# snuspl/parallax

Measured on NVIDIA H100. Metric: lm1b_words_per_sec, higher is better.
Workload: dtype bf16

## Files before the change

### parallax_b200/ops/csrc/kernels/gemm_tc.cu

```cuda
#include "wgmma.cuh"

namespace tc {

template <int BN, int STAGES>
__device__ __forceinline__ void mainloop(const CUtensorMap* tmap_a, const CUtensorMap* tmap_b,
                                         uint8_t* smem, uint64_t* full_bar, uint64_t* empty_bar,
                                         int k0, int num_kb, int m0, int n0, float* acc) {
  constexpr int A_BYTES = BM * BK * 2, B_BYTES = BN * BK * 2, STAGE_BYTES = A_BYTES + B_BYTES;
  const int wg = threadIdx.x >> 7;
  if (wg == 0) {
    if (threadIdx.x == 0) {
      for (int kb = 0; kb < num_kb; ++kb) {
        const int s = kb % STAGES;
        const uint32_t ph = (kb / STAGES) & 1;
        mbar_wait(&empty_bar[s], ph ^ 1);
        uint8_t* sa = smem + s * STAGE_BYTES;
        mbar_expect_tx(&full_bar[s], STAGE_BYTES);
        tma_load_2d(sa, tmap_a, &full_bar[s], k0 + kb * BK, m0);
        tma_load_2d(sa + A_BYTES, tmap_b, &full_bar[s], k0 + kb * BK, n0);
      }
    }
    return;
  }
  const int cw = wg - 1;
  const bool leader = (threadIdx.x & 127) == 0;
  for (int kb = 0; kb < num_kb; ++kb) {
    const int s = kb % STAGES;
    mbar_wait(&full_bar[s], (kb / STAGES) & 1);
    const uint32_t sa = smem_u32(smem + s * STAGE_BYTES);
    const uint64_t adesc = make_smem_desc(sa + cw * 64 * BK * 2);
    const uint64_t bdesc = make_smem_desc(sa + A_BYTES);
    wgmma_fence();
#pragma unroll
    for (int k = 0; k < BK / WG_K; ++k)
      wgmma_bf16<BN>(acc, adesc + (uint64_t)(k * 2), bdesc + (uint64_t)(k * 2),
                     (kb | k) != 0 ? 1u : 0u);
    wgmma_commit();
    wgmma_wait<1>();
    if (kb > 0 && leader) mbar_arrive(&empty_bar[(kb - 1) % STAGES]);
  }
  wgmma_wait<0>();
}

struct GemmArgs {
  __nv_bfloat16* C;
  const __nv_bfloat16* addend;
  float* ws;
  unsigned int* tickets;
  int M, N, K;
  int k_per_split;
};

__device__ __forceinline__ float2 bf16x2_to_float2(uint32_t w) {
  return make_float2(__uint_as_float(w << 16), __uint_as_float(w & 0xffff0000u));
}
__device__ __forceinline__ uint32_t float2_to_bf16x2(float a, float b) {
  __nv_bfloat162 h = __floats2bfloat162_rn(a, b);
  return *reinterpret_cast<uint32_t*>(&h);
}

__device__ __forceinline__ void cluster_sync_all() {
  asm volatile("barrier.cluster.arrive.release.aligned;\n"
               "barrier.cluster.wait.acquire.aligned;" ::: "memory");
}

template <int BN, int STAGES, bool CLUSTER>
__global__ void __launch_bounds__(THREADS, 1)
px_gemm_tc_kernel(const __grid_constant__ CUtensorMap tmap_a,
                  const __grid_constant__ CUtensorMap tmap_b, GemmArgs g) {
  extern __shared__ __align__(1024) uint8_t smem_raw[];
  uint8_t* smem = reinterpret_cast<uint8_t*>(((uintptr_t)smem_raw + 1023) & ~(uintptr_t)1023);
  constexpr int STAGE_BYTES = BM * BK * 2 + BN * BK * 2;
  uint64_t* full_bar = reinterpret_cast<uint64_t*>(smem + STAGES * STAGE_BYTES);
  uint64_t* empty_bar = full_bar + STAGES;
  __shared__ unsigned int s_last;

  const int n_tile = blockIdx.x, m_tile = blockIdx.y, split = blockIdx.z;

  if (threadIdx.x == 0) {
    asm volatile("prefetch.tensormap [%0];" ::"l"(&tmap_a) : "memory");
    asm volatile("prefetch.tensormap [%0];" ::"l"(&tmap_b) : "memory");
    for (int s = 0; s < STAGES; ++s) { mbar_init(&full_bar[s], 1); mbar_init(&empty_bar[s], 2); }
    asm volatile("fence.mbarrier_init.release.cluster;" ::: "memory");
  }
  __syncthreads();

  float acc[BN / 2];
  mainloop<BN, STAGES>(&tmap_a, &tmap_b, smem, full_bar, empty_bar, split * g.k_per_split,
                       g.k_per_split / BK, m_tile * BM, n_tile * BN, acc);

  if (threadIdx.x >= 128) {
    const int t = threadIdx.x - 128, lane = t & 31;
    const int lrow = (t >> 5) * 16 + (lane >> 2);
    const int lcol = (lane & 3) * 2;
    const bool splitk = gridDim.z > 1;
    if (CLUSTER) {
      consumer_sync();
      float* park = reinterpret_cast<float*>(smem);
#pragma unroll
      for (int j = 0; j < BN / 8; ++j)
#pragma unroll
        for (int h = 0; h < 2; ++h)
          *reinterpret_cast<float2*>(park + (size_t)(lrow + 8 * h) * (BN + 4) + j * 8 + lcol) =
              make_float2(acc[j * 4 + 2 * h], acc[j * 4 + 2 * h + 1]);
    } else {
#pragma unroll
      for (int h = 0; h < 2; ++h) {
        const int row = m_tile * BM + lrow + 8 * h;
        if (row >= g.M) continue;
        const size_t base = (size_t)row * g.N + (size_t)n_tile * BN + lcol;
#pragma unroll
        for (int j = 0; j < BN / 8; ++j) {
          const size_t off = base + j * 8;
          float2 v = make_float2(acc[j * 4 + 2 * h], acc[j * 4 + 2 * h + 1]);
          if (splitk) {
            atomicAdd(reinterpret_cast<float2*>(g.ws + off), v);
          } else {
            if (g.addend) {
              const float2 a = bf16x2_to_float2(*reinterpret_cast<const uint32_t*>(g.addend + off));
              v.x += a.x; v.y += a.y;
            }
            *reinterpret_cast<uint32_t*>(g.C + off) = float2_to_bf16x2(v.x, v.y);
          }
        }
      }
    }
  }
  __syncthreads();
  if (CLUSTER) {
    uint32_t crank, csize;
    asm volatile("mov.u32 %0, %%cluster_ctarank;" : "=r"(crank));
    asm volatile("mov.u32 %0, %%cluster_nctarank;" : "=r"(csize));
    cluster_sync_all();
    const int rows_per = BM / (int)csize;
    const int nvec = rows_per * BN / 4;
    const uint32_t my_base = smem_u32(smem);
    for (int v = threadIdx.x; v < nvec; v += blockDim.x) {
      const int rr = (int)crank * rows_per + (v * 4) / BN, cc = (v * 4) % BN;
      const uint32_t off_b = (uint32_t)(((size_t)rr * (BN + 4) + cc) * 4);
      float4 acc4 = make_float4(0.f, 0.f, 0.f, 0.f);
      for (uint32_t p = 0; p < csize; ++p) {
        uint32_t raddr;
        asm volatile("mapa.shared::cluster.u32 %0, %1, %2;" : "=r"(raddr) : "r"(my_base + off_b), "r"(p));
        float4 x;
        asm volatile("ld.shared::cluster.v4.f32 {%0,%1,%2,%3}, [%4];"
                     : "=f"(x.x), "=f"(x.y), "=f"(x.z), "=f"(x.w) : "r"(raddr) : "memory");
        acc4.x += x.x; acc4.y += x.y; acc4.z += x.z; acc4.w += x.w;
      }
      const int row = m_tile * BM + rr;
      if (row < g.M) {
        const size_t off = (size_t)row * g.N + (size_t)n_tile * BN + cc;
        if (g.addend) {
          const uint2 a2 = *reinterpret_cast<const uint2*>(g.addend + off);
          const float2 lo = bf16x2_to_float2(a2.x), hi = bf16x2_to_float2(a2.y);
          acc4.x += lo.x; acc4.y += lo.y; acc4.z += hi.x; acc4.w += hi.y;
        }
        *reinterpret_cast<uint2*>(g.C + off) =
            make_uint2(float2_to_bf16x2(acc4.x, acc4.y), float2_to_bf16x2(acc4.z, acc4.w));
      }
    }
    cluster_sync_all();
    return;
  }
  if (gridDim.z > 1) {
    __threadfence();
    __syncthreads();
    const unsigned int tile_id = m_tile * gridDim.x + n_tile;
    if (threadIdx.x == 0) s_last = (atomicAdd(&g.tickets[tile_id], 1u) == gridDim.z - 1) ? 1u : 0u;
    __syncthreads();
    if (s_last) {
      __threadfence();
      for (int idx = threadIdx.x; idx < BM * BN / 8; idx += blockDim.x) {
        const int rr = idx / (BN / 8), cc = (idx % (BN / 8)) * 8;
        const int row = m_tile * BM + rr;
        if (row >= g.M) continue;
        const size_t off = (size_t)row * g.N + (size_t)n_tile * BN + cc;
        float f[8];
        const uint4 lo = __ldcg(reinterpret_cast<const uint4*>(g.ws + off));
        const uint4 hi = __ldcg(reinterpret_cast<const uint4*>(g.ws + off + 4));
        f[0] = __uint_as_float(lo.x); f[1] = __uint_as_float(lo.y); f[2] = __uint_as_float(lo.z);
        f[3] = __uint_as_float(lo.w); f[4] = __uint_as_float(hi.x); f[5] = __uint_as_float(hi.y);
        f[6] = __uint_as_float(hi.z); f[7] = __uint_as_float(hi.w);
        if (g.addend) {
          float a[8];
          Vec16<__nv_bfloat16>::unpack(ld_v4(g.addend + off), a);
#pragma unroll
          for (int j = 0; j < 8; ++j) f[j] += a[j];
        }
        st_v4(g.C + off, Vec16<__nv_bfloat16>::pack(f));
        __stcg(reinterpret_cast<uint4*>(g.ws + off), make_uint4(0, 0, 0, 0));
        __stcg(reinterpret_cast<uint4*>(g.ws + off + 4), make_uint4(0, 0, 0, 0));
      }
      if (threadIdx.x == 0) g.tickets[tile_id] = 0;
    }
  }
}


template <int BN, int STAGES>
constexpr int smem_bytes() { return STAGES * (BM * BK * 2 + BN * BK * 2) + 1024 + 256; }

}

extern "C" {

int px_gemm_tc(const void* A, const void* B, void* C, const void* addend, float* ws,
               unsigned int* tickets, int M, int N, int K, int splits, int bn, int cluster,
               cudaStream_t stream) {
  using namespace tc;
  if (M % BM || K % BK || (bn != 64 && bn != 128) || N % bn) return -1;
  if (splits < 1 || K % (splits * BK)) return -2;
  if (cluster && (splits < 2 || splits > 16 || (BM % splits) != 0)) return -4;
  if (splits > 1 && !cluster && (!ws || !tickets)) return -3;
  CUtensorMap ta, tb;
  int rc = make_tmap(&ta, A, M, K, BM);
  if (rc) return rc;
  rc = make_tmap(&tb, B, N, K, bn);
  if (rc) return rc;
  GemmArgs g;
  g.C = (__nv_bfloat16*)C; g.addend = (const __nv_bfloat16*)addend; g.ws = ws;
  g.tickets = tickets; g.M = M; g.N = N; g.K = K; g.k_per_split = K / splits;
  dim3 grid(N / bn, M / BM, splits);
  constexpr int STAGES = 4;
  if (cluster) {
    cudaLaunchConfig_t cfg = {};
    cfg.gridDim = grid; cfg.blockDim = dim3(THREADS); cfg.stream = stream;
    cudaLaunchAttribute at[1];
    at[0].id = cudaLaunchAttributeClusterDimension;
    at[0].val.clusterDim.x = 1; at[0].val.clusterDim.y = 1; at[0].val.clusterDim.z = splits;
    cfg.attrs = at; cfg.numAttrs = 1;
    cudaError_t e;
    if (bn == 128) {
      constexpr int SMEM = smem_bytes<128, STAGES>();
      static bool setc128 = false;
      if (!setc128) {
        cudaFuncSetAttribute(px_gemm_tc_kernel<128, STAGES, true>,
                             cudaFuncAttributeMaxDynamicSharedMemorySize, SMEM);
        cudaFuncSetAttribute(px_gemm_tc_kernel<128, STAGES, true>,
                             cudaFuncAttributeNonPortableClusterSizeAllowed, 1);
        setc128 = true;
      }
      cfg.dynamicSmemBytes = SMEM;
      e = cudaLaunchKernelEx(&cfg, px_gemm_tc_kernel<128, STAGES, true>, ta, tb, g);
    } else {
      constexpr int SMEM = smem_bytes<64, STAGES>();
      static bool setc64 = false;
      if (!setc64) {
        cudaFuncSetAttribute(px_gemm_tc_kernel<64, STAGES, true>,
                             cudaFuncAttributeMaxDynamicSharedMemorySize, SMEM);
        cudaFuncSetAttribute(px_gemm_tc_kernel<64, STAGES, true>,
                             cudaFuncAttributeNonPortableClusterSizeAllowed, 1);
        setc64 = true;
      }
      cfg.dynamicSmemBytes = SMEM;
      e = cudaLaunchKernelEx(&cfg, px_gemm_tc_kernel<64, STAGES, true>, ta, tb, g);
    }
    return e == cudaSuccess ? (int)cudaGetLastError() : (int)e;
  }
  if (bn == 128) {
    constexpr int SMEM = smem_bytes<128, STAGES>();
    static bool set128 = false;
    if (!set128) {
      cudaFuncSetAttribute(px_gemm_tc_kernel<128, STAGES, false>,
                           cudaFuncAttributeMaxDynamicSharedMemorySize, SMEM);
      set128 = true;
    }
    px_gemm_tc_kernel<128, STAGES, false><<<grid, THREADS, SMEM, stream>>>(ta, tb, g);
  } else {
    constexpr int SMEM = smem_bytes<64, STAGES>();
    static bool set64 = false;
    if (!set64) {
      cudaFuncSetAttribute(px_gemm_tc_kernel<64, STAGES, false>,
                           cudaFuncAttributeMaxDynamicSharedMemorySize, SMEM);
      set64 = true;
    }
    px_gemm_tc_kernel<64, STAGES, false><<<grid, THREADS, SMEM, stream>>>(ta, tb, g);
  }
  return (int)cudaGetLastError();
}

}
```

### parallax_b200/ops/csrc/kernels/lstm_softmax.cu

```cuda
#include "common.cuh"

template <typename T> __device__ __forceinline__ float to_f(T v);
template <> __device__ __forceinline__ float to_f<float>(float v) { return v; }
template <> __device__ __forceinline__ float to_f<__nv_bfloat16>(__nv_bfloat16 v) { return __bfloat162float(v); }
template <typename T> __device__ __forceinline__ T from_f(float v);
template <> __device__ __forceinline__ float from_f<float>(float v) { return v; }
template <> __device__ __forceinline__ __nv_bfloat16 from_f<__nv_bfloat16>(float v) { return __float2bfloat16_rn(v); }

__device__ __forceinline__ float sigmoidf_(float x) { return 1.f / (1.f + __expf(-x)); }
__device__ __forceinline__ float tanhf_(float x) {
  const float e = __expf(-2.f * fabsf(x));
  const float t = (1.f - e) / (1.f + e);
  return copysignf(t, x);
}

template <typename T>
__global__ void __launch_bounds__(256)
px_lstm_cell_fwd_kernel(const T* __restrict__ gates, const float* __restrict__ c_prev,
                        T* __restrict__ act, float* __restrict__ c_new, T* __restrict__ m,
                        int B, int S, float forget_bias) {
  const int total = B * S;
  for (int idx = blockIdx.x * blockDim.x + threadIdx.x; idx < total;
       idx += gridDim.x * blockDim.x) {
    const int b = idx / S, s = idx - b * S;
    const size_t g0 = (size_t)b * 4 * S + s;
    const float si = sigmoidf_(to_f(gates[g0]));
    const float tj = tanhf_(to_f(gates[g0 + S]));
    const float sf = sigmoidf_(to_f(gates[g0 + 2 * S]) + forget_bias);
    const float so = sigmoidf_(to_f(gates[g0 + 3 * S]));
    const float c = sf * c_prev[idx] + si * tj;
    c_new[idx] = c;
    m[idx] = from_f<T>(so * tanhf_(c));
    act[g0] = from_f<T>(si);
    act[g0 + S] = from_f<T>(tj);
    act[g0 + 2 * S] = from_f<T>(sf);
    act[g0 + 3 * S] = from_f<T>(so);
  }
}

template <typename T>
__global__ void __launch_bounds__(256)
px_lstm_cell_bwd_kernel(const T* __restrict__ dm, float* __restrict__ dc,
                        const T* __restrict__ act, const float* __restrict__ c_prev,
                        const float* __restrict__ c_new, T* __restrict__ dgates, int B, int S) {
  const int total = B * S;
  for (int idx = blockIdx.x * blockDim.x + threadIdx.x; idx < total;
       idx += gridDim.x * blockDim.x) {
    const int b = idx / S, s = idx - b * S;
    const size_t g0 = (size_t)b * 4 * S + s;
    const float si = to_f(act[g0]), tj = to_f(act[g0 + S]), sf = to_f(act[g0 + 2 * S]),
                so = to_f(act[g0 + 3 * S]);
    const float tc = tanhf_(c_new[idx]);
    const float dmv = to_f(dm[idx]);
    const float dcv = dc[idx] + dmv * so * (1.f - tc * tc);
    dgates[g0] = from_f<T>(dcv * tj * si * (1.f - si));
    dgates[g0 + S] = from_f<T>(dcv * si * (1.f - tj * tj));
    dgates[g0 + 2 * S] = from_f<T>(dcv * c_prev[idx] * sf * (1.f - sf));
    dgates[g0 + 3 * S] = from_f<T>(dmv * tc * so * (1.f - so));
    dc[idx] = dcv * sf;
  }
}

template <typename T, int ITEMS, bool DOT>
__global__ void __launch_bounds__(256)
px_sampled_softmax_kernel(T* __restrict__ logits, const float* __restrict__ true_dot,
                          const float* __restrict__ adj_true,
                          const float* __restrict__ adj_samp,
                          const long long* __restrict__ targets, const long long* __restrict__ sampled,
                          float* __restrict__ loss, float* __restrict__ dtrue, int N, int S,
                          const T* __restrict__ h, const T* __restrict__ w_true, int P) {
  const int row = blockIdx.x;
  if (row >= N) return;
  __shared__ float s_red[8];
  __shared__ float s_bcast;
  T* x = logits + (size_t)row * S;
  const long long tgt = targets[row];
  float tl;
  if (DOT) {
    __shared__ float s_dot[8];
    const T* hr = h + (size_t)row * P;
    const T* wr = w_true + (size_t)row * P;
    float part = 0.f;
    for (int k = threadIdx.x; k < P; k += 256) part += to_f(hr[k]) * to_f(wr[k]);
    part = warp_sum(part);
    if ((threadIdx.x & 31) == 0) s_dot[threadIdx.x >> 5] = part;
    __syncthreads();
    float t = 0.f;
#pragma unroll
    for (int k = 0; k < 8; ++k) t += s_dot[k];
    tl = t + adj_true[row];
  } else {
    tl = true_dot[row] + adj_true[row];
  }
  float v[ITEMS];
  float mx = tl;
#pragma unroll
  for (int k = 0; k < ITEMS; ++k) {
    const int j = k * 256 + threadIdx.x;
    float a = -INFINITY;
    if (j < S) {
      a = to_f(x[j]) + adj_samp[j];
      if (sampled[j] == tgt) a = -INFINITY;
    }
    v[k] = a;
    mx = fmaxf(mx, a);
  }
  for (int o = 16; o > 0; o >>= 1) mx = fmaxf(mx, __shfl_xor_sync(0xffffffffu, mx, o));
  if ((threadIdx.x & 31) == 0) s_red[threadIdx.x >> 5] = mx;
  __syncthreads();
  if (threadIdx.x < 32) {
    float t = threadIdx.x < 8 ? s_red[threadIdx.x] : -INFINITY;
    for (int o = 4; o > 0; o >>= 1) t = fmaxf(t, __shfl_xor_sync(0xffffffffu, t, o));
    if (threadIdx.x == 0) s_bcast = t;
  }
  __syncthreads();
  mx = s_bcast;
  float sum = 0.f;
#pragma unroll
  for (int k = 0; k < ITEMS; ++k) { v[k] = __expf(v[k] - mx); sum += v[k]; }
  sum = warp_sum(sum);
  __syncthreads();
  if ((threadIdx.x & 31) == 0) s_red[threadIdx.x >> 5] = sum;
  __syncthreads();
  if (threadIdx.x < 32) {
    float t = threadIdx.x < 8 ? s_red[threadIdx.x] : 0.f;
    t = warp_sum(t);
    if (threadIdx.x == 0) s_bcast = t + __expf(tl - mx);
  }
  __syncthreads();
  const float denom = s_bcast;
  const float inv = 1.f / denom;
#pragma unroll
  for (int k = 0; k < ITEMS; ++k) {
    const int j = k * 256 + threadIdx.x;
    if (j < S) x[j] = from_f<T>(v[k] * inv);
  }
  if (threadIdx.x == 0) {
    loss[row] = (mx + __logf(denom)) - tl;
    dtrue[row] = __expf(tl - mx) * inv - 1.f;
  }
}

// ... 163 lines not shown
```

### parallax_b200/ops/fused.py

```python
import ctypes

import torch

from . import lib as _lib, check as _check, register_signatures

_vp, _i, _f = ctypes.c_void_p, ctypes.c_int, ctypes.c_float
register_signatures({
    "px_lstm_cell_fwd": (_i, [_vp, _vp, _vp, _vp, _vp, _i, _i, _f, _i, _vp]),
    "px_lstm_cell_bwd": (_i, [_vp, _vp, _vp, _vp, _vp, _vp, _i, _i, _i, _vp]),
    "px_sampled_softmax": (_i, [_vp, _vp, _vp, _vp, _vp, _vp, _vp, _vp, _i, _i, _i, _vp]),
    "px_sampled_softmax_dot": (_i, [_vp, _vp, _vp, _i, _vp, _vp, _vp, _vp, _vp, _vp, _i, _i, _i,
                                    _vp]),
    "px_ssm_bwd": (_i, [_vp, _vp, _vp, _vp, _i, _vp, _vp, _f, _vp, _vp, _vp, _i, _vp, _i, _i, _i,
                        _vp]),
})
_DT = {torch.float32: 0, torch.bfloat16: 1}


def _p(t):
    return _vp(t.data_ptr())


def _stream():
    return _vp(torch.cuda.current_stream().cuda_stream)


def _count(n=1):
    from ..parallel import nvops
    nvops.launches["n"] += n


def _acc(t):
    return t if t.dtype == torch.float64 else t.float()


def lstm_layer_reference(x, Wx, Wh, bias, W_P, c0, h0, forget_bias=1.0):
    T, Bsz, E = x.shape
    S = W_P.shape[0]
    xw = torch.addmm(bias, x.reshape(T * Bsz, E), Wx).view(T, Bsz, 4 * S)
    c, h, outs = _acc(c0), h0, []
    for t in range(T):
        gates = _acc(torch.addmm(xw[t], h, Wh))
        i, j, f, o = gates.split(S, dim=1)
        c = torch.sigmoid(f + forget_bias) * c + torch.sigmoid(i) * torch.tanh(j)
        m = (torch.sigmoid(o) * torch.tanh(c)).to(x.dtype)
        h = m @ W_P
        outs.append(h)
    return torch.stack(outs), c, h


class _LSTMLayerFn(torch.autograd.Function):

    @staticmethod
    def forward(ctx, x, W, Wh, bias, W_P, c0, h0, forget_bias):
        L = _lib()
        T, Bsz, E = x.shape
        S, P = W_P.shape
        dt = x.dtype
        dev = x.device
        x = x.contiguous()
        stacked = Wh is None
        ctx.stacked = stacked
        ctx.param_refs = (W, bias, W_P)
        if stacked:
            Wx, Wh = W.detach()[:E], W.detach()[E:]
        else:
            Wx = W
        if any(ctx.needs_input_grad):
            from . import sinks
            cur = torch.cuda.current_stream(dev)
            ws = sinks.side_stream(dev)
            ws.wait_stream(cur)
            with torch.cuda.stream(ws):
                ctx.WPT = W_P.detach().t().contiguous()
                ctx.WPT_ev = torch.cuda.Event()
                ctx.WPT_ev.record(ws)
            ctx.WPT.record_stream(cur)
        xw = torch.addmm(bias, x.view(T * Bsz, E), Wx).view(T, Bsz, 4 * S)
        act = torch.empty(T, Bsz, 4 * S, dtype=dt, device=dev)
        c_all = torch.empty(T + 1, Bsz, S, dtype=torch.float32, device=dev)
        m_all = torch.empty(T, Bsz, S, dtype=dt, device=dev)
        h_all = torch.empty(T + 1, Bsz, P, dtype=dt, device=dev)
        c_all[0].copy_(c0)
        h_all[0].copy_(h0)
        st = _stream()
        for t in range(T):
            gpre = xw[t].addmm_(h_all[t], Wh)
            _check(L.px_lstm_cell_fwd(_p(gpre), _p(c_all[t]), _p(act[t]),
                                      _p(c_all[t + 1]), _p(m_all[t]), Bsz, S,
                                      float(forget_bias), _DT[dt], st), "lstm_cell_fwd")
            torch.mm(m_all[t], W_P, out=h_all[t + 1])
        _count(T)
        ctx.save_for_backward(x, Wx, Wh, W_P, act, c_all, m_all, h_all)
        ctx.dims = (T, Bsz, E, S, P)
        return h_all[1:], c_all[T].clone(), h_all[T].clone()

    @staticmethod
    def backward(ctx, dH, dcT, dhT):
        from . import sinks
        L = _lib()
        x, Wx, Wh, W_P, act, c_all, m_all, h_all = ctx.saved_tensors
        T, Bsz, E, S, P = ctx.dims
        stacked = ctx.stacked
        W_ref, bias_ref, WP_ref = ctx.param_refs
        dt, dev = x.dtype, x.device
        dH = dH.contiguous()
        dgates = torch.empty(T, Bsz, 4 * S, dtype=dt, device=dev)
        dh_tot = torch.empty(T, Bsz, P, dtype=dt, device=dev)
        dc = torch.zeros(Bsz, S, dtype=torch.float32, device=dev) if dcT is None \
            else dcT.float().clone()
        dh_rec = None if dhT is None else dhT.to(dt)
        dm = torch.empty(Bsz, S, dtype=dt, device=dev)
        cur = torch.cuda.current_stream(dev)
        cur.wait_event(ctx.WPT_ev)
        WPT = ctx.WPT
        from . import gemm as _gemm
        use_tc = (dt == torch.bfloat16 and Bsz % 128 == 0 and P % 64 == 0 and
                  (4 * S) % 1024 == 0 and Wh.is_contiguous())
        WhT = None if use_tc else Wh.t().contiguous()
        st = _stream()

        def sink_of(ref, shape):
            s_ = sinks.get(ref)
            if s_ is not None and s_.dtype == dt and tuple(s_.shape) == tuple(shape):
                return s_, True
            return torch.empty(shape, dtype=dt, device=dev), False
        if stacked:
            dW, w_sunk = sink_of(W_ref, (E + P, 4 * S))
            dWx_o, dWh_o = dW[:E], dW[E:]
        else:
            dWx_o, w_sunk = sink_of(W_ref, (E, 4 * S))
            dWh_o = torch.empty(P, 4 * S, dtype=dt, device=dev)
        dbias_o, b_sunk = sink_of(bias_ref, (4 * S,))
        dWP_o, p_sunk = sink_of(WP_ref, (S, P))
        ws = sinks.side_stream(dev)
        ws2 = sinks.side_stream(dev, 1)
        if dh_rec is None:
            dh_tot[T - 1].copy_(dH[T - 1])
        else:
            torch.add(dH[T - 1], dh_rec, out=dh_tot[T - 1])
        for t in range(T - 1, -1, -1):
            torch.mm(dh_tot[t], WPT, out=dm)
            _check(L.px_lstm_cell_bwd(_p(dm), _p(dc), _p(act[t]), _p(c_all[t]),
                                      _p(c_all[t + 1]), _p(dgates[t]), Bsz, S, _DT[dt], st),
                   "lstm_cell_bwd")
            if t > 0:
                if use_tc:
                    _gemm.gemm_tn(dgates[t], Wh, addend=dH[t - 1], splits=8, bn=64,
                                  out=dh_tot[t - 1])
                else:
                    torch.addmm(dH[t - 1], dgates[t], WhT, out=dh_tot[t - 1])
            else:
                dh_rec = _gemm.gemm_tn(dgates[0], Wh, splits=8, bn=64) if use_tc \
                    else torch.mm(dgates[0], WhT)
        _count(T)
        dg2 = dgates.view(T * Bsz, 4 * S)
        ws2.wait_stream(cur)
        with torch.cuda.stream(ws2):
            torch.sum(dg2, 0, out=dbias_o)
        ev_b = torch.cuda.Event()
        ev_b.record(ws2)
        dgates.record_stream(ws2)
        dbias_o.record_stream(ws2)
        dx = (dg2 @ Wx.t()).view(T, Bsz, E)
        ws.wait_stream(cur)
        with torch.cuda.stream(ws):
            torch.mm(h_all[:T].reshape(-1, P).t(), dg2, out=dWh_o)
            torch.mm(x.reshape(-1, E).t(), dg2, out=dWx_o)
            torch.mm(m_all.reshape(-1, S).t(), dh_tot.view(-1, P), out=dWP_o)
        ev = torch.cuda.Event()
        ev.record(ws)
        for t_ in (dgates, dh_tot, x, h_all, m_all, dWh_o, dWx_o, dbias_o, dWP_o):
            t_.record_stream(ws)
        outs, plain = [], False
        for ref, o, sunk, e_ in ((W_ref, dW if stacked else dWx_o, w_sunk, ev),
                                 (bias_ref, dbias_o, b_sunk, ev_b), (WP_ref, dWP_o, p_sunk, ev)):
            if sunk:
                sinks.deliver(ref, e_)
                outs.append(None)
            else:
                outs.append(o)
                plain = True
        if plain or not stacked:
            cur.wait_event(ev)
            cur.wait_event(ev_b)
        dW_out, dbias, dW_P = outs
        return dx, dW_out, None if stacked else dWh_o, dbias, dW_P, dc, dh_rec, None


def lstm_layer(x, Wx, Wh, bias, W_P, c0, h0, forget_bias=1.0):
    if x.is_cuda and x.dtype in _DT:
        return _LSTMLayerFn.apply(x, Wx, Wh, bias, W_P, c0, h0, forget_bias)
    return lstm_layer_reference(x, Wx, Wh, bias, W_P, c0, h0, forget_bias)


def lstm_layer_stacked(x, W, bias, W_P, c0, h0, forget_bias=1.0):
    E = x.shape[-1]
    if x.is_cuda and x.dtype in _DT:
        return _LSTMLayerFn.apply(x, W, None, bias, W_P, c0, h0, forget_bias)
    return lstm_layer_reference(x, W[:E], W[E:], bias, W_P, c0, h0, forget_bias)


def sampled_softmax_reference(inputs, true_w, samp_w, true_b, samp_b, logq_true,
                              logq_samp, targets, sampled):
    true_logits = _acc((inputs * true_w).sum(-1)) + _acc(true_b) - logq_true
    samp_logits = _acc(inputs @ samp_w.t()) + (_acc(samp_b) - logq_samp)
    hits = targets.unsqueeze(1) == sampled.unsqueeze(0)
    samp_logits = samp_logits.masked_fill(hits, float("-inf"))
    lse = torch.logsumexp(torch.cat([true_logits.unsqueeze(1), samp_logits], 1), 1)
    return lse - true_logits


class _SampledSoftmaxFn(torch.autograd.Function):
    @staticmethod
    def forward(ctx, inputs, true_w, samp_w, true_b, samp_b, logq_true, logq_samp,
                targets, sampled):
        L = _lib()
        N, S = inputs.shape[0], samp_w.shape[0]
        dt = inputs.dtype
        logits = inputs @ samp_w.t()
        true_dot = (inputs.float() * true_w.float()).sum(-1)
        adj_t = (true_b.float() - logq_true).contiguous()
        adj_s = (samp_b.float() - logq_samp).contiguous()
        loss = torch.empty(N, dtype=torch.float32, device=inputs.device)
        dtrue = torch.empty(N, dtype=torch.float32, device=inputs.device)
        tg = targets.to(torch.int64).contiguous()
        sm = sampled.to(torch.int64).contiguous()
        _check(L.px_sampled_softmax(_p(logits), _p(true_dot), _p(adj_t), _p(adj_s), _p(tg),
                                    _p(sm), _p(loss), _p(dtrue), N, S, _DT[dt], _stream()),
               "sampled_softmax")
        _count(1)
        ctx.save_for_backward(inputs, true_w, samp_w, logits, dtrue)
        return loss

    @staticmethod
    def backward(ctx, g):
        inputs, true_w, samp_w, probs, dtrue = ctx.saved_tensors
# ... 133 lines not shown
```

### parallax_b200/ops/gemm.py

```python
import ctypes

import torch

from .. import consts
from . import lib as _lib, check as _check, register_signatures

_vp, _i = ctypes.c_void_p, ctypes.c_int
register_signatures({
    "px_gemm_tc": (_i, [_vp, _vp, _vp, _vp, _vp, _vp, _i, _i, _i, _i, _i, _i, _vp]),
})

_ws_cache = {}


def _workspace(M, N, device):
    key = (M, N, str(device))
    w = _ws_cache.get(key)
    if w is None:
        w = (torch.zeros(M, N, dtype=torch.float32, device=device),
             torch.zeros(max(1, (M // 128) * (N // 64)), dtype=torch.int32, device=device))
        _ws_cache[key] = w
    return w


def pick_splits(M, N, K, bn=128, sms=consts.NUM_SMS):
    tiles = (M // 128) * (N // bn)
    s = max(1, min(K // 256, sms // max(tiles, 1)))
    while s > 1 and K % (s * 64) != 0:
        s -= 1
    return s


def supported(A, Bt):
    return (A.is_cuda and A.dtype == torch.bfloat16 and Bt.dtype == torch.bfloat16 and
            A.dim() == 2 and Bt.dim() == 2 and A.is_contiguous() and Bt.is_contiguous() and
            A.shape[0] % 128 == 0 and A.shape[1] % 64 == 0 and Bt.shape[0] % 64 == 0 and
            A.data_ptr() % 16 == 0 and Bt.data_ptr() % 16 == 0)


def gemm_tn(A, Bt, addend=None, splits=None, out=None, bn=None, cluster=True):
    M, K = A.shape
    N = Bt.shape[0]
    assert Bt.shape[1] == K
    if bn is None:
        bn = 128 if N % 128 == 0 else 64
    if splits is None:
        splits = pick_splits(M, N, K, bn)
    if out is None:
        out = torch.empty(M, N, dtype=torch.bfloat16, device=A.device)
    cluster = bool(cluster) and 2 <= splits <= 16 and 128 % splits == 0
    ws = tk = None
    if splits > 1 and not cluster:
        ws, tk = _workspace(M, N, A.device)
    from ..parallel import nvops
    nvops.launches["n"] += 1
    rc = _lib().px_gemm_tc(
        _vp(A.data_ptr()), _vp(Bt.data_ptr()), _vp(out.data_ptr()),
        _vp(addend.data_ptr()) if addend is not None else _vp(0),
        _vp(ws.data_ptr()) if ws is not None else _vp(0),
        _vp(tk.data_ptr()) if tk is not None else _vp(0), M, N, K, splits, bn,
        1 if cluster else 0, _vp(torch.cuda.current_stream().cuda_stream))
    _check(rc, "gemm_tc")
    return out
```

Measured before the change: 1.861 million.

## Fuse LSTM backward projection GEMM with cell backward and chain steps via PDL

Replaces the per-timestep torch.mm (dh·W_P) plus separate cell-backward kernel with one cluster split-K kernel. Its epilogue reduces partials across the cluster in distributed shared memory and applies the LSTM cell backward directly. The step kernel and the recurrent dgates·Wh GEMM are launched with programmatic dependent launch: weight tiles load and cell tensors prefetch to L2 before griddepcontrol.wait, overlapping launch latency and prologue across the serial chain. The forward pass skips materializing the transposed W_P when this path is used. The cost is more complex synchronization and correctness reliance on PDL ordering.

```diff
diff --git a/parallax_b200/ops/csrc/kernels/gemm_tc.cu b/parallax_b200/ops/csrc/kernels/gemm_tc.cu
--- a/parallax_b200/ops/csrc/kernels/gemm_tc.cu
+++ b/parallax_b200/ops/csrc/kernels/gemm_tc.cu
@@ -1,8 +1,16 @@
 #include "wgmma.cuh"
+#include "lstm_cell.cuh"
 
 namespace tc {
 
-template <int BN, int STAGES>
+__device__ __forceinline__ void griddep_wait() {
+  asm volatile("griddepcontrol.wait;" ::: "memory");
+}
+__device__ __forceinline__ void griddep_launch_dependents() {
+  asm volatile("griddepcontrol.launch_dependents;" ::: "memory");
+}
+
+template <int BN, int STAGES, bool PDL = false>
 __device__ __forceinline__ void mainloop(const CUtensorMap* tmap_a, const CUtensorMap* tmap_b,
                                          uint8_t* smem, uint64_t* full_bar, uint64_t* empty_bar,
                                          int k0, int num_kb, int m0, int n0, float* acc) {
@@ -10,14 +18,26 @@
   const int wg = threadIdx.x >> 7;
   if (wg == 0) {
     if (threadIdx.x == 0) {
+      int pre = 0;
+      if constexpr (PDL) {
+        pre = num_kb < STAGES ? num_kb : STAGES;
+        for (int kb = 0; kb < pre; ++kb) {
+          mbar_expect_tx(&full_bar[kb], STAGE_BYTES);
+          tma_load_2d(smem + kb * STAGE_BYTES + A_BYTES, tmap_b, &full_bar[kb], k0 + kb * BK, n0);
+        }
+        griddep_wait();
+        griddep_launch_dependents();
+      }
       for (int kb = 0; kb < num_kb; ++kb) {
         const int s = kb % STAGES;
         const uint32_t ph = (kb / STAGES) & 1;
-        mbar_wait(&empty_bar[s], ph ^ 1);
         uint8_t* sa = smem + s * STAGE_BYTES;
-        mbar_expect_tx(&full_bar[s], STAGE_BYTES);
+        if (kb >= pre) {
+          mbar_wait(&empty_bar[s], ph ^ 1);
+          mbar_expect_tx(&full_bar[s], STAGE_BYTES);
+        }
         tma_load_2d(sa, tmap_a, &full_bar[s], k0 + kb * BK, m0);
-        tma_load_2d(sa + A_BYTES, tmap_b, &full_bar[s], k0 + kb * BK, n0);
+        if (kb >= pre) tma_load_2d(sa + A_BYTES, tmap_b, &full_bar[s], k0 + kb * BK, n0);
       }
     }
     return;
@@ -64,7 +84,35 @@
                "barrier.cluster.wait.acquire.aligned;" ::: "memory");
 }
 
-template <int BN, int STAGES, bool CLUSTER>
+template <int BN>
+__device__ __forceinline__ void park_partial(const float* acc, uint8_t* smem) {
+  const int t = threadIdx.x - 128, lane = t & 31;
+  const int lrow = (t >> 5) * 16 + (lane >> 2);
+  const int lcol = (lane & 3) * 2;
+  consumer_sync();
+  float* park = reinterpret_cast<float*>(smem);
+#pragma unroll
+  for (int j = 0; j < BN / 8; ++j)
+#pragma unroll
+    for (int h = 0; h < 2; ++h)
+      *reinterpret_cast<float2*>(park + (size_t)(lrow + 8 * h) * (BN + 4) + j * 8 + lcol) =
+          make_float2(acc[j * 4 + 2 * h], acc[j * 4 + 2 * h + 1]);
+}
+
+__device__ __forceinline__ float4 cluster_sum4(uint32_t my_base, uint32_t off_b, uint32_t csize) {
+  float4 acc4 = make_float4(0.f, 0.f, 0.f, 0.f);
+  for (uint32_t p = 0; p < csize; ++p) {
+    uint32_t raddr;
+    asm volatile("mapa.shared::cluster.u32 %0, %1, %2;" : "=r"(raddr) : "r"(my_base + off_b), "r"(p));
+    float4 x;
+    asm volatile("ld.shared::cluster.v4.f32 {%0,%1,%2,%3}, [%4];"
+                 : "=f"(x.x), "=f"(x.y), "=f"(x.z), "=f"(x.w) : "r"(raddr) : "memory");
+    acc4.x += x.x; acc4.y += x.y; acc4.z += x.z; acc4.w += x.w;
+  }
+  return acc4;
+}
+
+template <int BN, int STAGES, bool CLUSTER, bool PDL = false>
 __global__ void __launch_bounds__(THREADS, 1)
 px_gemm_tc_kernel(const __grid_constant__ CUtensorMap tmap_a,
                   const __grid_constant__ CUtensorMap tmap_b, GemmArgs g) {
@@ -85,9 +133,15 @@
   }
   __syncthreads();
 
+  if constexpr (PDL) {
+    if (threadIdx.x != 0) {
+      griddep_wait();
+      griddep_launch_dependents();
+    }
+  }
   float acc[BN / 2];
-  mainloop<BN, STAGES>(&tmap_a, &tmap_b, smem, full_bar, empty_bar, split * g.k_per_split,
-                       g.k_per_split / BK, m_tile * BM, n_tile * BN, acc);
+  mainloop<BN, STAGES, PDL>(&tmap_a, &tmap_b, smem, full_bar, empty_bar, split * g.k_per_split,
+                            g.k_per_split / BK, m_tile * BM, n_tile * BN, acc);
 
   if (threadIdx.x >= 128) {
     const int t = threadIdx.x - 128, lane = t & 31;
@@ -95,14 +149,7 @@
     const int lcol = (lane & 3) * 2;
     const bool splitk = gridDim.z > 1;
     if (CLUSTER) {
-      consumer_sync();
-      float* park = reinterpret_cast<float*>(smem);
-#pragma unroll
-      for (int j = 0; j < BN / 8; ++j)
-#pragma unroll
-        for (int h = 0; h < 2; ++h)
-          *reinterpret_cast<float2*>(park + (size_t)(lrow + 8 * h) * (BN + 4) + j * 8 + lcol) =
-              make_float2(acc[j * 4 + 2 * h], acc[j * 4 + 2 * h + 1]);
+      park_partial<BN>(acc, smem);
     } else {
 #pragma unroll
       for (int h = 0; h < 2; ++h) {
@@ -138,15 +185,7 @@
     for (int v = threadIdx.x; v < nvec; v += blockDim.x) {
       const int rr = (int)crank * rows_per + (v * 4) / BN, cc = (v * 4) % BN;
       const uint32_t off_b = (uint32_t)(((size_t)rr * (BN + 4) + cc) * 4);
-      float4 acc4 = make_float4(0.f, 0.f, 0.f, 0.f);
-      for (uint32_t p = 0; p < csize; ++p) {
-        uint32_t raddr;
-        asm volatile("mapa.shared::cluster.u32 %0, %1, %2;" : "=r"(raddr) : "r"(my_base + off_b), "r"(p));
-        float4 x;
-        asm volatile("ld.shared::cluster.v4.f32 {%0,%1,%2,%3}, [%4];"
-                     : "=f"(x.x), "=f"(x.y), "=f"(x.z), "=f"(x.w) : "r"(raddr) : "memory");
-        acc4.x += x.x; acc4.y += x.y; acc4.z += x.z; acc4.w += x.w;
-      }
+      float4 acc4 = cluster_sum4(my_base, off_b, csize);
       const int row = m_tile * BM + rr;
       if (row < g.M) {
         const size_t off = (size_t)row * g.N + (size_t)n_tile * BN + cc;
@@ -196,18 +235,137 @@
   }
 }
 
+struct StepArgs {
+  const __nv_bfloat16* act;
+  const float* c_prev;
+  const float* c_new;
+  float* dc;
+  __nv_bfloat16* dgates;
+  int S;
+  int k_per_split;
+};
+
+__device__ __forceinline__ void ld_bf16x4(const __nv_bfloat16* p, float* f) {
+  const uint2 w = *reinterpret_cast<const uint2*>(p);
+  const float2 lo = bf16x2_to_float2(w.x), hi = bf16x2_to_float2(w.y);
+  f[0] = lo.x; f[1] = lo.y; f[2] = hi.x; f[3] = hi.y;
+}
+__device__ __forceinline__ void st_bf16x4(__nv_bfloat16* p, const float* f) {
+  *reinterpret_cast<uint2*>(p) = make_uint2(float2_to_bf16x2(f[0], f[1]), float2_to_bf16x2(f[2], f[3]));
+}
+__device__ __forceinline__ void ld_f32x4(const float* p, float* f) {
+  const float4 v = *reinterpret_cast<const float4*>(p);
+  f[0] = v.x; f[1] = v.y; f[2] = v.z; f[3] = v.w;
+}
+
+template <int BN, int STAGES>
+__global__ void __launch_bounds__(THREADS, 1)
+px_lstm_bwd_step_kernel(const __grid_constant__ CUtensorMap tmap_a,
+                        const __grid_constant__ CUtensorMap tmap_b, StepArgs g) {
+  extern __shared__ __align__(1024) uint8_t smem_raw[];
+  uint8_t* smem = reinterpret_cast<uint8_t*>(((uintptr_t)smem_raw + 1023) & ~(uintptr_t)1023);
+  constexpr int STAGE_BYTES = BM * BK * 2 + BN * BK * 2;
+  uint64_t* full_bar = reinterpret_cast<uint64_t*>(smem + STAGES * STAGE_BYTES);
+  uint64_t* empty_bar = full_bar + STAGES;
+  const int n_tile = blockIdx.x, m_tile = blockIdx.y, split = blockIdx.z;
+  const int S = g.S;
+
+  if (threadIdx.x == 0) {
+    asm volatile("prefetch.tensormap [%0];" ::"l"(&tmap_a) : "memory");
+    asm volatile("prefetch.tensormap [%0];" ::"l"(&tmap_b) : "memory");
+    for (int s = 0; s < STAGES; ++s) { mbar_init(&full_bar[s], 1); mbar_init(&empty_bar[s], 2); }
+    asm volatile("fence.mbarrier_init.release.cluster;" ::: "memory");
+  }
+  __syncthreads();
+
+  uint32_t crank, csize;
+  asm volatile("mov.u32 %0, %%cluster_ctarank;" : "=r"(crank));
+  asm volatile("mov.u32 %0, %%cluster_nctarank;" : "=r"(csize));
+  const int rows_per = BM / (int)csize;
+  if (threadIdx.x != 0) {
+    constexpr int ACT_LINES = BN * 2 / 128, CELL_LINES = BN * 4 / 128;
+    constexpr int LINES = 4 * ACT_LINES + 3 * CELL_LINES;
+    for (int i = threadIdx.x - 1; i < rows_per * LINES; i += blockDim.x - 1) {
+      const size_t row = (size_t)m_tile * BM + (int)crank * rows_per + i / LINES;
+      const int l = i % LINES, s0 = n_tile * BN;
+      const void* a;
+      if (l < 4 * ACT_LINES)
+        a = g.act + row * 4 * S + (size_t)(l / ACT_LINES) * S + s0 + (l % ACT_LINES) * 64;
+      else {
+        const int c = (l - 4 * ACT_LINES) / CELL_LINES, o = (l - 4 * ACT_LINES) % CELL_LINES * 32;
+        const float* base = c == 0 ? g.c_prev : c == 1 ? g.c_new : g.dc;
+        a = base + row * S + s0 + o;
+      }
+      asm volatile("prefetch.global.L2 [%0];" ::"l"(a));
+    }
+    griddep_wait();
+    griddep_launch_dependents();
+  }
+  float acc[BN / 2];
+  mainloop<BN, STAGES, true>(&tmap_a, &tmap_b, smem, full_bar, empty_bar, split * g.k_per_split,
+                             g.k_per_split / BK, m_tile * BM, n_tile * BN, acc);
+  if (threadIdx.x >= 128) park_partial<BN>(acc, smem);
+  __syncthreads();
+
+  cluster_sync_all();
+  const int nvec = rows_per * BN / 4;
+  const uint32_t my_base = smem_u32(smem);
+  for (int v = threadIdx.x; v < nvec; v += blockDim.x) {
+    const int rr = (int)crank * rows_per + (v * 4) / BN, u = (v * 4) % BN;
+    const size_t row = (size_t)m_tile * BM + rr;
+    const int s = n_tile * BN + u;
+    const size_t cell = row * S + s, gate = row * 4 * S + s;
+    float a[4][4], cp[4], cn[4], dc[4], out[4][4];
+#pragma unroll
+    for (int q = 0; q < 4; ++q) ld_bf16x4(g.act + gate + (size_t)q * S, a[q]);
+    ld_f32x4(g.c_prev + cell, cp);
+    ld_f32x4(g.c_new + cell, cn);
+    ld_f32x4(g.dc + cell, dc);
+    const float4 x = cluster_sum4(my_base, (uint32_t)(((size_t)rr * (BN + 4) + u) * 4), csize);
+    const float dm[4] = {x.x, x.y, x.z, x.w};
+#pragma unroll
+    for (int e = 0; e < 4; ++e) {
+      const LstmCellBwd r = lstm_cell_bwd(a[0][e], a[1][e], a[2][e], a[3][e], cp[e], cn[e], dm[e],
+                                          dc[e]);
+      out[0][e] = r.di; out[1][e] = r.dj; out[2][e] = r.df; out[3][e] = r.dout;
+      dc[e] = r.dc;
+    }
+    *reinterpret_cast<float4*>(g.dc + cell) = make_float4(dc[0], dc[1], dc[2], dc[3]);
+#pragma unroll
+    for (int q = 0; q < 4; ++q) st_bf16x4(g.dgates + gate + (size_t)q * S, out[q]);
+  }
+  cluster_sync_all();
+}
+
 
 template <int BN, int STAGES>
 constexpr int smem_bytes() { return STAGES * (BM * BK * 2 + BN * BK * 2) + 1024 + 256; }
 
-}
-
-extern "C" {
-
-int px_gemm_tc(const void* A, const void* B, void* C, const void* addend, float* ws,
-               unsigned int* tickets, int M, int N, int K, int splits, int bn, int cluster,
-               cudaStream_t stream) {
-  using namespace tc;
+template <auto Kern, typename... Args>
+static int launch_cluster(int smem, dim3 grid, int splits, bool pdl, cudaStream_t stream,
+                          const Args&... args) {
+  static bool attrs_set = false;
+  if (!attrs_set) {
+    cudaFuncSetAttribute(Kern, cudaFuncAttributeMaxDynamicSharedMemorySize, smem);
+    cudaFuncSetAttribute(Kern, cudaFuncAttributeNonPortableClusterSizeAllowed, 1);
+    attrs_set = true;
+  }
+  cudaLaunchConfig_t cfg = {};
+  cfg.gridDim = grid; cfg.blockDim = dim3(THREADS); cfg.dynamicSmemBytes = smem;
+  cfg.stream = stream;
+  cudaLaunchAttribute at[2];
+  at[0].id = cudaLaunchAttributeClusterDimension;
+  at[0].val.clusterDim.x = 1; at[0].val.clusterDim.y = 1; at[0].val.clusterDim.z = splits;
+  at[1].id = cudaLaunchAttributeProgrammaticStreamSerialization;
+  at[1].val.programmaticStreamSerializationAllowed = 1;
+  cfg.attrs = at; cfg.numAttrs = pdl ? 2 : 1;
+  const cudaError_t e = cudaLaunchKernelEx(&cfg, Kern, args...);
+  return e == cudaSuccess ? (int)cudaGetLastError() : (int)e;
+}
+
+static int gemm_tc(const void* A, const void* B, void* C, const void* addend, float* ws,
+                   unsigned int* tickets, int M, int N, int K, int splits, int bn, int cluster,
+                   bool pdl, cudaStream_t stream) {
   if (M % BM || K % BK || (bn != 64 && bn != 128) || N % bn) return -1;
   if (splits < 1 || K % (splits * BK)) return -2;
   if (cluster && (splits < 2 || splits > 16 || (BM % splits) != 0)) return -4;
@@ -223,39 +381,15 @@
   dim3 grid(N / bn, M / BM, splits);
   constexpr int STAGES = 4;
   if (cluster) {
-    cudaLaunchConfig_t cfg = {};
-    cfg.gridDim = grid; cfg.blockDim = dim3(THREADS); cfg.stream = stream;
-    cudaLaunchAttribute at[1];
-    at[0].id = cudaLaunchAttributeClusterDimension;
-    at[0].val.clusterDim.x = 1; at[0].val.clusterDim.y = 1; at[0].val.clusterDim.z = splits;
-    cfg.attrs = at; cfg.numAttrs = 1;
-    cudaError_t e;
-    if (bn == 128) {
-      constexpr int SMEM = smem_bytes<128, STAGES>();
-      static bool setc128 = false;
-      if (!setc128) {
-        cudaFuncSetAttribute(px_gemm_tc_kernel<128, STAGES, true>,
-                             cudaFuncAttributeMaxDynamicSharedMemorySize, SMEM);
-        cudaFuncSetAttribute(px_gemm_tc_kernel<128, STAGES, true>,
-                             cudaFuncAttributeNonPortableClusterSizeAllowed, 1);
-        setc128 = true;
-      }
-      cfg.dynamicSmemBytes = SMEM;
-      e = cudaLaunchKernelEx(&cfg, px_gemm_tc_kernel<128, STAGES, true>, ta, tb, g);
-    } else {
-      constexpr int SMEM = smem_bytes<64, STAGES>();
-      static bool setc64 = false;
-      if (!setc64) {
-        cudaFuncSetAttribute(px_gemm_tc_kernel<64, STAGES, true>,
-                             cudaFuncAttributeMaxDynamicSharedMemorySize, SMEM);
-        cudaFuncSetAttribute(px_gemm_tc_kernel<64, STAGES, true>,
-                             cudaFuncAttributeNonPortableClusterSizeAllowed, 1);
-        setc64 = true;
-      }
-      cfg.dynamicSmemBytes = SMEM;
-      e = cudaLaunchKernelEx(&cfg, px_gemm_tc_kernel<64, STAGES, true>, ta, tb, g);
-    }
-    return e == cudaSuccess ? (int)cudaGetLastError() : (int)e;
+    if (bn == 128)
+      return pdl ? launch_cluster<px_gemm_tc_kernel<128, STAGES, true, true>>(
+                       smem_bytes<128, STAGES>(), grid, splits, true, stream, ta, tb, g)
+                 : launch_cluster<px_gemm_tc_kernel<128, STAGES, true>>(
+                       smem_bytes<128, STAGES>(), grid, splits, false, stream, ta, tb, g);
+    return pdl ? launch_cluster<px_gemm_tc_kernel<64, STAGES, true, true>>(
+                     smem_bytes<64, STAGES>(), grid, splits, true, stream, ta, tb, g)
+               : launch_cluster<px_gemm_tc_kernel<64, STAGES, true>>(
+                     smem_bytes<64, STAGES>(), grid, splits, false, stream, ta, tb, g);
   }
   if (bn == 128) {
     constexpr int SMEM = smem_bytes<128, STAGES>();
@@ -279,4 +413,39 @@
   return (int)cudaGetLastError();
 }
 
-}
+constexpr int STEP_BN = 64, STEP_STAGES = 4;
+
+}
+
+extern "C" {
+
+int px_gemm_tc(const void* A, const void* B, void* C, const void* addend, float* ws,
+               unsigned int* tickets, int M, int N, int K, int splits, int bn, int cluster,
+               cudaStream_t stream) {
+  return tc::gemm_tc(A, B, C, addend, ws, tickets, M, N, K, splits, bn, cluster, false, stream);
+}
+
+int px_gemm_tc_pdl(const void* A, const void* B, void* C, const void* addend, int M, int N, int K,
+                   int splits, int bn, cudaStream_t stream) {
+  return tc::gemm_tc(A, B, C, addend, nullptr, nullptr, M, N, K, splits, bn, 1, true, stream);
+}
+
+int px_lstm_bwd_step(const void* dh, const void* W_P, const void* act, const float* c_prev,
+                     const float* c_new, float* dc, void* dgates, int B, int S, int P, int splits,
+                     cudaStream_t stream) {
+  using namespace tc;
+  if (B <= 0 || B % BM || S % STEP_BN || P % BK) return -1;
+  if (splits < 1 || splits > 8 || (P / BK) % splits || BM % splits) return -2;
+  CUtensorMap ta, tb;
+  int rc = make_tmap(&ta, dh, B, P, BM);
+  if (rc) return rc;
+  if ((rc = make_tmap(&tb, W_P, S, P, STEP_BN))) return rc;
+  StepArgs g;
+  g.act = (const __nv_bfloat16*)act; g.c_prev = c_prev; g.c_new = c_new; g.dc = dc;
+  g.dgates = (__nv_bfloat16*)dgates; g.S = S; g.k_per_split = P / splits;
+  return launch_cluster<px_lstm_bwd_step_kernel<STEP_BN, STEP_STAGES>>(
+      smem_bytes<STEP_BN, STEP_STAGES>(), dim3(S / STEP_BN, B / BM, splits), splits, true, stream,
+      ta, tb, g);
+}
+
+}
diff --git a/parallax_b200/ops/csrc/kernels/lstm_cell.cuh b/parallax_b200/ops/csrc/kernels/lstm_cell.cuh
--- /dev/null
+++ b/parallax_b200/ops/csrc/kernels/lstm_cell.cuh
@@ -0,0 +1,36 @@
+#pragma once
+
+__device__ __forceinline__ float sigmoidf_(float x) { return 1.f / (1.f + __expf(-x)); }
+__device__ __forceinline__ float tanhf_(float x) {
+  const float e = __expf(-2.f * fabsf(x));
+  const float t = (1.f - e) / (1.f + e);
+  return copysignf(t, x);
+}
+
+struct LstmCellFwd { float si, tj, sf, so, c, m; };
+__device__ __forceinline__ LstmCellFwd lstm_cell_fwd(float gi, float gj, float gf, float go,
+                                                     float c_prev, float forget_bias) {
+  LstmCellFwd r;
+  r.si = sigmoidf_(gi);
+  r.tj = tanhf_(gj);
+  r.sf = sigmoidf_(gf + forget_bias);
+  r.so = sigmoidf_(go);
+  r.c = r.sf * c_prev + r.si * r.tj;
+  r.m = r.so * tanhf_(r.c);
+  return r;
+}
+
+struct LstmCellBwd { float di, dj, df, dout, dc; };
+__device__ __forceinline__ LstmCellBwd lstm_cell_bwd(float si, float tj, float sf, float so,
+                                                     float c_prev, float c_new, float dmv,
+                                                     float dc_in) {
+  LstmCellBwd r;
+  const float tc = tanhf_(c_new);
+  const float dcv = dc_in + dmv * so * (1.f - tc * tc);
+  r.di = dcv * tj * si * (1.f - si);
+  r.dj = dcv * si * (1.f - tj * tj);
+  r.df = dcv * c_prev * sf * (1.f - sf);
+  r.dout = dmv * tc * so * (1.f - so);
+  r.dc = dcv * sf;
+  return r;
+}
diff --git a/parallax_b200/ops/csrc/kernels/lstm_softmax.cu b/parallax_b200/ops/csrc/kernels/lstm_softmax.cu
--- a/parallax_b200/ops/csrc/kernels/lstm_softmax.cu
+++ b/parallax_b200/ops/csrc/kernels/lstm_softmax.cu
@@ -1,4 +1,5 @@
 #include "common.cuh"
+#include "lstm_cell.cuh"
 
 template <typename T> __device__ __forceinline__ float to_f(T v);
 template <> __device__ __forceinline__ float to_f<float>(float v) { return v; }
@@ -6,13 +7,6 @@
 template <typename T> __device__ __forceinline__ T from_f(float v);
 template <> __device__ __forceinline__ float from_f<float>(float v) { return v; }
 template <> __device__ __forceinline__ __nv_bfloat16 from_f<__nv_bfloat16>(float v) { return __float2bfloat16_rn(v); }
-
-__device__ __forceinline__ float sigmoidf_(float x) { return 1.f / (1.f + __expf(-x)); }
-__device__ __forceinline__ float tanhf_(float x) {
-  const float e = __expf(-2.f * fabsf(x));
-  const float t = (1.f - e) / (1.f + e);
-  return copysignf(t, x);
-}
 
 template <typename T>
 __global__ void __launch_bounds__(256)
@@ -24,17 +18,15 @@
        idx += gridDim.x * blockDim.x) {
     const int b = idx / S, s = idx - b * S;
     const size_t g0 = (size_t)b * 4 * S + s;
-    const float si = sigmoidf_(to_f(gates[g0]));
-    const float tj = tanhf_(to_f(gates[g0 + S]));
-    const float sf = sigmoidf_(to_f(gates[g0 + 2 * S]) + forget_bias);
-    const float so = sigmoidf_(to_f(gates[g0 + 3 * S]));
-    const float c = sf * c_prev[idx] + si * tj;
-    c_new[idx] = c;
-    m[idx] = from_f<T>(so * tanhf_(c));
-    act[g0] = from_f<T>(si);
-    act[g0 + S] = from_f<T>(tj);
-    act[g0 + 2 * S] = from_f<T>(sf);
-    act[g0 + 3 * S] = from_f<T>(so);
+    const LstmCellFwd r = lstm_cell_fwd(to_f(gates[g0]), to_f(gates[g0 + S]),
+                                        to_f(gates[g0 + 2 * S]), to_f(gates[g0 + 3 * S]),
+                                        c_prev[idx], forget_bias);
+    c_new[idx] = r.c;
+    m[idx] = from_f<T>(r.m);
+    act[g0] = from_f<T>(r.si);
+    act[g0 + S] = from_f<T>(r.tj);
+    act[g0 + 2 * S] = from_f<T>(r.sf);
+    act[g0 + 3 * S] = from_f<T>(r.so);
   }
 }
 
@@ -48,16 +40,14 @@
        idx += gridDim.x * blockDim.x) {
     const int b = idx / S, s = idx - b * S;
     const size_t g0 = (size_t)b * 4 * S + s;
-    const float si = to_f(act[g0]), tj = to_f(act[g0 + S]), sf = to_f(act[g0 + 2 * S]),
-                so = to_f(act[g0 + 3 * S]);
-    const float tc = tanhf_(c_new[idx]);
-    const float dmv = to_f(dm[idx]);
-    const float dcv = dc[idx] + dmv * so * (1.f - tc * tc);
-    dgates[g0] = from_f<T>(dcv * tj * si * (1.f - si));
-    dgates[g0 + S] = from_f<T>(dcv * si * (1.f - tj * tj));
-    dgates[g0 + 2 * S] = from_f<T>(dcv * c_prev[idx] * sf * (1.f - sf));
-    dgates[g0 + 3 * S] = from_f<T>(dmv * tc * so * (1.f - so));
-    dc[idx] = dcv * sf;
+    const LstmCellBwd r = lstm_cell_bwd(to_f(act[g0]), to_f(act[g0 + S]), to_f(act[g0 + 2 * S]),
+                                        to_f(act[g0 + 3 * S]), c_prev[idx], c_new[idx],
+                                        to_f(dm[idx]), dc[idx]);
+    dgates[g0] = from_f<T>(r.di);
+    dgates[g0 + S] = from_f<T>(r.dj);
+    dgates[g0 + 2 * S] = from_f<T>(r.df);
+    dgates[g0 + 3 * S] = from_f<T>(r.dout);
+    dc[idx] = r.dc;
   }
 }
 
diff --git a/parallax_b200/ops/fused.py b/parallax_b200/ops/fused.py
--- a/parallax_b200/ops/fused.py
+++ b/parallax_b200/ops/fused.py
@@ -8,6 +8,7 @@
 register_signatures({
     "px_lstm_cell_fwd": (_i, [_vp, _vp, _vp, _vp, _vp, _i, _i, _f, _i, _vp]),
     "px_lstm_cell_bwd": (_i, [_vp, _vp, _vp, _vp, _vp, _vp, _i, _i, _i, _vp]),
+    "px_lstm_bwd_step": (_i, [_vp, _vp, _vp, _vp, _vp, _vp, _vp, _i, _i, _i, _i, _vp]),
     "px_sampled_softmax": (_i, [_vp, _vp, _vp, _vp, _vp, _vp, _vp, _vp, _i, _i, _i, _vp]),
     "px_sampled_softmax_dot": (_i, [_vp, _vp, _vp, _i, _vp, _vp, _vp, _vp, _vp, _vp, _i, _i, _i,
                                     _vp]),
@@ -49,6 +50,18 @@
     return torch.stack(outs), c, h
 
 
+def _step_chain(dt, Bsz, S, P, Wh, W_P):
+    return (dt == torch.bfloat16 and Bsz % 128 == 0 and P % 64 == 0 and (4 * S) % 1024 == 0 and
+            Wh.is_contiguous() and W_P.is_contiguous())
+
+
+def _splits(kb, most):
+    s = most
+    while kb % s:
+        s //= 2
+    return s
+
+
 class _LSTMLayerFn(torch.autograd.Function):
 
     @staticmethod
@@ -66,7 +79,8 @@
             Wx, Wh = W.detach()[:E], W.detach()[E:]
         else:
             Wx = W
-        if any(ctx.needs_input_grad):
+        ctx.chain = _step_chain(dt, Bsz, S, P, Wh, W_P)
+        if any(ctx.needs_input_grad) and not ctx.chain:
             from . import sinks
             cur = torch.cuda.current_stream(dev)
             ws = sinks.side_stream(dev)
@@ -110,11 +124,13 @@
         dc = torch.zeros(Bsz, S, dtype=torch.float32, device=dev) if dcT is None \
             else dcT.float().clone()
         dh_rec = None if dhT is None else dhT.to(dt)
-        dm = torch.empty(Bsz, S, dtype=dt, device=dev)
+        chain = ctx.chain
         cur = torch.cuda.current_stream(dev)
-        cur.wait_event(ctx.WPT_ev)
-        WPT = ctx.WPT
         from . import gemm as _gemm
+        if not chain:
+            dm = torch.empty(Bsz, S, dtype=dt, device=dev)
+            cur.wait_event(ctx.WPT_ev)
+            WPT = ctx.WPT
         use_tc = (dt == torch.bfloat16 and Bsz % 128 == 0 and P % 64 == 0 and
                   (4 * S) % 1024 == 0 and Wh.is_contiguous())
         WhT = None if use_tc else Wh.t().contiguous()
@@ -139,20 +155,32 @@
             dh_tot[T - 1].copy_(dH[T - 1])
         else:
             torch.add(dH[T - 1], dh_rec, out=dh_tot[T - 1])
-        for t in range(T - 1, -1, -1):
-            torch.mm(dh_tot[t], WPT, out=dm)
-            _check(L.px_lstm_cell_bwd(_p(dm), _p(dc), _p(act[t]), _p(c_all[t]),
-                                      _p(c_all[t + 1]), _p(dgates[t]), Bsz, S, _DT[dt], st),
-                   "lstm_cell_bwd")
-            if t > 0:
-                if use_tc:
+        if chain:
+            sp_b = _splits(P // 64, 4)
+            for t in range(T - 1, -1, -1):
+                _check(L.px_lstm_bwd_step(_p(dh_tot[t]), _p(W_P), _p(act[t]), _p(c_all[t]),
+                                          _p(c_all[t + 1]), _p(dc), _p(dgates[t]), Bsz, S, P,
+                                          sp_b, st), "lstm_bwd_step")
+                if t > 0:
                     _gemm.gemm_tn(dgates[t], Wh, addend=dH[t - 1], splits=8, bn=64,
-                                  out=dh_tot[t - 1])
+                                  out=dh_tot[t - 1], pdl=True)
                 else:
-                    torch.addmm(dH[t - 1], dgates[t], WhT, out=dh_tot[t - 1])
-            else:
-                dh_rec = _gemm.gemm_tn(dgates[0], Wh, splits=8, bn=64) if use_tc \
-                    else torch.mm(dgates[0], WhT)
+                    dh_rec = _gemm.gemm_tn(dgates[0], Wh, splits=8, bn=64, pdl=True)
+        else:
+            for t in range(T - 1, -1, -1):
+                torch.mm(dh_tot[t], WPT, out=dm)
+                _check(L.px_lstm_cell_bwd(_p(dm), _p(dc), _p(act[t]), _p(c_all[t]),
+                                          _p(c_all[t + 1]), _p(dgates[t]), Bsz, S, _DT[dt], st),
+                       "lstm_cell_bwd")
+                if t > 0:
+                    if use_tc:
+                        _gemm.gemm_tn(dgates[t], Wh, addend=dH[t - 1], splits=8, bn=64,
+                                      out=dh_tot[t - 1])
+                    else:
+                        torch.addmm(dH[t - 1], dgates[t], WhT, out=dh_tot[t - 1])
+                else:
+                    dh_rec = _gemm.gemm_tn(dgates[0], Wh, splits=8, bn=64) if use_tc \
+                        else torch.mm(dgates[0], WhT)
         _count(T)
         dg2 = dgates.view(T * Bsz, 4 * S)
         ws2.wait_stream(cur)
diff --git a/parallax_b200/ops/gemm.py b/parallax_b200/ops/gemm.py
--- a/parallax_b200/ops/gemm.py
+++ b/parallax_b200/ops/gemm.py
@@ -8,6 +8,7 @@
 _vp, _i = ctypes.c_void_p, ctypes.c_int
 register_signatures({
     "px_gemm_tc": (_i, [_vp, _vp, _vp, _vp, _vp, _vp, _i, _i, _i, _i, _i, _i, _vp]),
+    "px_gemm_tc_pdl": (_i, [_vp, _vp, _vp, _vp, _i, _i, _i, _i, _i, _vp]),
 })
 
 _ws_cache = {}
@@ -38,7 +39,7 @@
             A.data_ptr() % 16 == 0 and Bt.data_ptr() % 16 == 0)
 
 
-def gemm_tn(A, Bt, addend=None, splits=None, out=None, bn=None, cluster=True):
+def gemm_tn(A, Bt, addend=None, splits=None, out=None, bn=None, cluster=True, pdl=False):
     M, K = A.shape
     N = Bt.shape[0]
     assert Bt.shape[1] == K
@@ -54,6 +55,16 @@
         ws, tk = _workspace(M, N, A.device)
     from ..parallel import nvops
     nvops.launches["n"] += 1
+    if pdl:
+        if not cluster:
+            raise ValueError("gemm_tn: pdl needs the cluster schedule (2 <= splits <= 16, "
+                             "splits dividing 128), got splits=%d" % splits)
+        rc = _lib().px_gemm_tc_pdl(
+            _vp(A.data_ptr()), _vp(Bt.data_ptr()), _vp(out.data_ptr()),
+            _vp(addend.data_ptr()) if addend is not None else _vp(0), M, N, K, splits, bn,
+            _vp(torch.cuda.current_stream().cuda_stream))
+        _check(rc, "gemm_tc_pdl")
+        return out
     rc = _lib().px_gemm_tc(
         _vp(A.data_ptr()), _vp(Bt.data_ptr()), _vp(out.data_ptr()),
         _vp(addend.data_ptr()) if addend is not None else _vp(0),
```

New measurement: 1.874 million, median of 6. No clear change (+0.7%).
